# AnnaUshnova/tinyrenderder

Hardware: AMD Instinct MI355X
Metric: triangles/sec (+ Mpixels/sec) at 4096x4096; achieved HBM GB/s vs peak (higher is better)
Workload: dtype f64

## Files before the change

tinyrenderder_amd/csrc/kernels_bin.hip:

```cpp
#include <hip/hip_runtime.h>
#include "trgl_device.h"
#include "launch.h"

namespace {

__device__ __forceinline__ double dmin3(double a, double b, double c) { double m = a; if (b < m) m = b; if (c < m) m = c; return m; }
__device__ __forceinline__ double dmax3(double a, double b, double c) { double m = a; if (m < b) m = b; if (m < c) m = c; return m; }
__device__ __forceinline__ double dot4(const double* m, const double* v) {
    double sum = 0;
    sum += m[0] * v[0]; sum += m[1] * v[1]; sum += m[2] * v[2]; sum += m[3] * v[3];
    return sum;
}

__device__ __forceinline__ int wave_min_i(int v) {
    for (int o = 32; o; o >>= 1) { int t = __shfl_xor(v, o); v = t < v ? t : v; }
    return v;
}
__device__ __forceinline__ int wave_max_i(int v) {
    for (int o = 32; o; o >>= 1) { int t = __shfl_xor(v, o); v = t > v ? t : v; }
    return v;
}

constexpr int SCAN_THREADS = 256;

// ... 35 lines not shown
            if (++tx > tx1) { tx = tx0; ++row; ty = fp.il_tiles ? (uint32_t)il_nth_owned_from(fp, (int)ty0, (int)row) : ty0 + row; }
        }
    }
    unsigned long long big = __ballot(c > SMALL);
    const int lane = threadIdx.x & 63;
    while (big) {
        int src = __ffsll((long long)big) - 1;
        big &= big - 1;
        uint32_t cc = __shfl(c, src), oo = __shfl(o, src), ii = __shfl(i, src);
        uint32_t bx = __shfl(tb.x, src), by = __shfl(tb.y, src);
        const uint32_t qx0 = bx & 0x1fff, qy0 = (bx >> 16) & 0x1fff, qx1 = by & 0x1fff, qy1 = (by >> 16) & 0x1fff;
        ii |= (((bx >> 13) & 7u) | (((by >> 13) & 7u) << 3) | ((by >> 29) << 6)) << 25;
        uint32_t tx0 = qx0 >> 2, ty0 = qy0 >> 2, tx1 = qx1 >> 2;
        uint32_t wdt = tx1 - tx0 + 1;
        for (uint32_t k = lane; k < cc; k += 64) {
            uint32_t ty = fp.il_tiles ? (uint32_t)il_nth_owned_from(fp, (int)ty0, (int)(k / wdt)) : ty0 + k / wdt, tx = tx0 + k % wdt;
            put(oo + k, ty * tiles_x + tx, ii, tile_block_mask(tx, ty, qx0, qy0, qx1, qy1));
        }
    }
}

constexpr uint32_t SEG_MAX = 4096, SEG_MAX_GROUP = 16;

constexpr int SETUP_THREADS = 256;

__global__ __launch_bounds__(SETUP_THREADS) void k_setup(FrameParams fp, DrawDesc d, DrawDesc* __restrict__ draws_out, int draw_idx,
                                                         TriRec* __restrict__ recs, TriW* __restrict__ recs_w, uint32_t* __restrict__ cnt,
                                                         uint2* __restrict__ tilebox, DevStats* __restrict__ stats,
                                                         uint32_t* __restrict__ blk_sums, uint32_t blk_base,
                                                         uint32_t* __restrict__ seg_k, uint32_t* __restrict__ seg_v, uint32_t seg_S) {
    __shared__ __attribute__((aligned(16))) double s_buf[SETUP_THREADS * 16];
    if (blockIdx.x == 0 && threadIdx.x == 0) draws_out[draw_idx] = d;
    const uint32_t b0 = blockIdx.x * SETUP_THREADS;
    const uint32_t nb = min((uint32_t)SETUP_THREADS, d.n - b0);
    const uint32_t tid = threadIdx.x;
    const uint32_t i = b0 + tid;
    const bool in_range = tid < nb;

    const double* src = d.clip + (size_t)b0 * 12;
    if ((reinterpret_cast<uintptr_t>(src) & 15) == 0) {
        const double2* s2 = reinterpret_cast<const double2*>(src);
        double2* l2 = reinterpret_cast<double2*>(s_buf);
        typedef double f64x2 __attribute__((ext_vector_type(2)));
        for (uint32_t k = tid; k < nb * 6; k += SETUP_THREADS)
            *reinterpret_cast<f64x2*>(&l2[k]) = __builtin_nontemporal_load(reinterpret_cast<const f64x2*>(&s2[k]));
    } else {
        for (uint32_t k = tid; k < nb * 12; k += SETUP_THREADS) s_buf[k] = src[k];
    }
    __syncthreads();
    double v[12];
#pragma unroll
    for (int k = 0; k < 12; ++k) v[k] = in_range ? s_buf[tid * 12 + k] : 0.0;
    __syncthreads();

    int bx0 = INT_MAX, by0 = INT_MAX, bx1 = INT_MIN, by1 = INT_MIN;
    uint32_t ntiles = 0;
    bool large = false;
    uint2 tb = make_uint2(0, 0);
    TriRec r;
    {
        uint4* z4 = reinterpret_cast<uint4*>(&r);
#pragma unroll
        for (int k = 0; k < 8; ++k) z4[k] = make_uint4(0, 0, 0, 0);
    }
    if (in_range) {
        bool ok = !(v[3] <= 1e-12 || v[7] <= 1e-12 || v[11] <= 1e-12);
        double ndc[12];
#pragma unroll
        for (int q = 0; q < 3; ++q) {
#pragma unroll
            for (int k = 0; k < 3; ++k) ndc[4 * q + k] = v[4 * q + k] / v[4 * q + 3];
            ndc[4 * q + 3] = __builtin_isfinite(v[4 * q + 3]) ? 1.0 : __builtin_nan("");
        }
        bool zo0 = (ndc[2] < -1.0 || ndc[2] > 1.0), zo1 = (ndc[6] < -1.0 || ndc[6] > 1.0),
             zo2 = (ndc[10] < -1.0 || ndc[10] > 1.0);
        ok = ok && !(zo0 && zo1 && zo2);
#pragma unroll
        for (int k = 0; k < 12; ++k) ok = ok && __builtin_isfinite(ndc[k]);
        double sx[3], sy[3];
#pragma unroll
        for (int q = 0; q < 3; ++q) { sx[q] = dot4(fp.vp, ndc + 4 * q); sy[q] = dot4(fp.vp + 4, ndc + 4 * q); }
        double e1x = sx[1] - sx[0], e1y = sy[1] - sy[0], e2x = sx[2] - sx[0], e2y = sy[2] - sy[0];
// ... 8 lines not shown
            bx0 = min_x_px; by0 = min_y_px; bx1 = max_x_px; by1 = max_y_px;
            r.ax = sx[0]; r.ay = sy[0];
            r.s0x = sx[2] - sx[0]; r.s0y = sx[1] - sx[0];
            r.s1x = sy[2] - sy[0]; r.s1y = sy[1] - sy[0];
            r.uz = r.s0x * r.s1y - r.s0y * r.s1x;
            {
                const double BIG = 0x1p200, SMALL = 0x1p-250;
                bool ws = r.uz < 0.0 && !(fabs(r.uz) < 1e-12);
#pragma unroll
                for (int q = 0; q < 3; ++q) ws = ws && fabs(sx[q]) < BIG && fabs(sy[q]) < BIG;
                const double dl[4] = { r.s0x, r.s0y, r.s1x, r.s1y };
#pragma unroll
                for (int q = 0; q < 4; ++q) ws = ws && (dl[q] == 0.0 || fabs(dl[q]) >= SMALL);
                {
                    const double S = (fabs(r.s0x) + fabs(r.s0y)) + (fabs(r.s1x) + fabs(r.s1y));
                    const double rx = fmax(fabs(r.ax - ((double)bx0 + 0.5)), fabs(r.ax - ((double)bx1 + 0.5)));
                    const double ry = fmax(fabs(r.ay - ((double)by0 + 0.5)), fabs(r.ay - ((double)by1 + 0.5)));
                    ws = ws && 0x1p-40 * (S * S) * (rx + ry + 17.0 + S) < fabs(r.uz);
                }
                r.ruz = ws ? 1.0 / r.uz : 0.0;
            }
            r.z0 = ndc[2]; r.z1 = ndc[6]; r.z2 = ndc[10];
            r.bx0 = (uint16_t)bx0; r.by0 = (uint16_t)by0; r.bx1 = (uint16_t)bx1; r.by1 = (uint16_t)by1;
            r.color = d.colors ? d.colors[i] : 0xffffffffu;
            r.dl = ((uint32_t)draw_idx << 24) | i | (r.ruz == 0.0 ? TRGL_DL_LITERAL : 0u);
            r.c0 = -__builtin_inf(); r.g1 = 0.0; r.g2 = 0.0;
            if (r.ruz != 0.0) {
                const double zabs = dmax3(fabs(r.z0), fabs(r.z1), fabs(r.z2));
                const double dz1 = r.z1 - r.z0, dz2 = r.z2 - r.z0;
                const double h1 = (r.s1x * dz1 - r.s1y * dz2) * r.ruz, h2 = (r.s0y * dz2 - r.s0x * dz1) * r.ruz;
                const double rx = fmax(fabs(r.ax - ((double)bx0 + 0.5)), fabs(r.ax - ((double)bx1 + 0.5)));
                const double ry = fmax(fabs(r.ay - ((double)by0 + 0.5)), fabs(r.ay - ((double)by1 + 0.5)));
                const double Ssum = (fabs(r.s0x) + fabs(r.s0y)) + (fabs(r.s1x) + fabs(r.s1y));
                const double R = rx + ry + 1.0 + Ssum;
                const double mz = zabs * 0x1p-39 * (R * Ssum * fabs(r.ruz) + 1.0) + 0x1p-600;
                const bool okp = zabs < 0x1p1000 && R * fabs(h1) < 0x1p900 && R * fabs(h2) < 0x1p900 && mz < 0x1p1000;
                if (okp) { r.c0 = r.z0 - mz; r.g1 = h1; r.g2 = h2; }
            }
            if (d.kind != TRGL_SHADER_FLAT) {
                TriW w;
                w.iw0 = (fabs(v[3]) > 1e-12) ? (1.0 / v[3]) : 0.0;
                w.iw1 = (fabs(v[7]) > 1e-12) ? (1.0 / v[7]) : 0.0;
                w.iw2 = (fabs(v[11]) > 1e-12) ? (1.0 / v[11]) : 0.0;
                w.pad = 0.0;
                recs_w[d.first + i] = w;
            }
            int y_lo = max(by0, fp.strip_y0), y_hi = min(by1, fp.strip_y1 - 1);
            if (!(fabs(r.uz) < 1e-12) && y_lo <= y_hi) {
                uint32_t tx0 = bx0 >> TRGL_TILE_LOG2, tx1 = bx1 >> TRGL_TILE_LOG2;
                uint32_t ty0 = y_lo >> TRGL_TILE_LOG2, ty1 = y_hi >> TRGL_TILE_LOG2;
                const uint32_t rows = fp.il_tiles ? (uint32_t)(il_owned_below(fp, (int)ty1 + 1) - il_owned_below(fp, (int)ty0)) : ty1 - ty0 + 1;
                ntiles = (tx1 - tx0 + 1) * rows;
                tb = make_uint2(((uint32_t)bx0 >> TRGL_BLOCK_LOG2) | (((uint32_t)y_lo >> TRGL_BLOCK_LOG2) << 16),
                                ((uint32_t)bx1 >> TRGL_BLOCK_LOG2) | (((uint32_t)y_hi >> TRGL_BLOCK_LOG2) << 16));
                uint32_t zq = 0;
                if (r.c0 > -__builtin_inf()) {
                    const double zv = dmin3(r.c0, __builtin_fma(-r.s0y, r.g1, __builtin_fma(-r.s1y, r.g2, r.c0)),
                                            __builtin_fma(-r.s0x, r.g1, __builtin_fma(-r.s1x, r.g2, r.c0)));
                    const double t = (zv + 1.0) * 64.0 - 0x1p-20;
                    if (t >= 1.0) zq = t >= 127.0 ? 127u : (uint32_t)x86_cvttsd2si(floor(t));
                }
                tb.x |= (zq & 7u) << 13; tb.y |= ((zq >> 3) & 7u) << 13; tb.y |= (zq >> 6) << 29;
                large = ntiles != 0 && (bx1 - bx0 >= 64 || y_hi - y_lo >= 64);
            }
        }
        cnt[d.first + i] = ntiles;
        tilebox[d.first + i] = tb;
    }
    const uint32_t lane = tid & 63, wbase = tid & ~63u;
    {
        uint4* l4 = reinterpret_cast<uint4*>(s_buf);
        const uint4* r4 = reinterpret_cast<const uint4*>(&r);
#pragma unroll
        for (int c = 0; c < 8; ++c) l4[tid * 8 + (c ^ (tid & 7))] = r4[c];
        const unsigned long long keep = __ballot(ntiles != 0);
        __builtin_amdgcn_wave_barrier();
        uint4* dst = reinterpret_cast<uint4*>(recs + d.first + b0 + wbase);
#pragma unroll
        for (int it = 0; it < 8; ++it) {
            const uint32_t k = lane + 64u * it, t = k >> 3, c = k & 7;
            if ((keep >> t) & 1ull) {
                typedef uint32_t u32x4 __attribute__((ext_vector_type(4)));
                __builtin_nontemporal_store(*reinterpret_cast<const u32x4*>(&l4[(wbase + t) * 8 + (c ^ (t & 7))]), reinterpret_cast<u32x4*>(&dst[k]));
            }
        }
    }
    {
        const unsigned long long lit = __ballot(ntiles != 0 && r.ruz == 0.0);
        if (lit && lane == 0) atomicAdd(&stats->literal_tris, (unsigned long long)__popcll(lit));
        const unsigned long long lrg = __ballot(large);
        if (lrg && lane == 0) atomicAdd(&stats->large_tris, (unsigned long long)__popcll(lrg));
// ... 1 lines not shown
    int wx0 = wave_min_i(bx0), wy0 = wave_min_i(by0), wx1 = wave_max_i(bx1), wy1 = wave_max_i(by1);
    if ((threadIdx.x & 63) == 0 && wx0 != INT_MAX) {
        if (wx0 < __builtin_nontemporal_load(&stats->min_x)) atomicMin(&stats->min_x, wx0);
        if (wy0 < __builtin_nontemporal_load(&stats->min_y)) atomicMin(&stats->min_y, wy0);
        if (wx1 > __builtin_nontemporal_load(&stats->max_x)) atomicMax(&stats->max_x, wx1);
        if (wy1 > __builtin_nontemporal_load(&stats->max_y)) atomicMax(&stats->max_y, wy1);
    }
    uint32_t tot;
    const uint32_t off = block_excl_scan(ntiles, reinterpret_cast<uint32_t*>(s_buf), &tot);
    if (tid == 0) blk_sums[blk_base + blockIdx.x] = tot;
    if (seg_S && tot && tot <= seg_S) {
        __syncthreads();
        uint32_t* const s_k = reinterpret_cast<uint32_t*>(s_buf);
        uint32_t* const s_v = s_k + SEG_MAX;
        block_pairs(fp, fp.tiles_x, d.first + i, ntiles, tb, off, [&](uint32_t j, uint32_t key, uint32_t iz, uint32_t m) { s_k[j] = key | (m << 16); s_v[j] = iz; });
        __syncthreads();
        uint4* const kq = reinterpret_cast<uint4*>(seg_k + (size_t)(blk_base + blockIdx.x) * seg_S);
        uint4* const vq = reinterpret_cast<uint4*>(seg_v + (size_t)(blk_base + blockIdx.x) * seg_S);
        for (uint32_t q = tid; 4 * q < tot; q += SETUP_THREADS) {
            kq[q] = *reinterpret_cast<const uint4*>(s_k + 4 * q);
            vq[q] = *reinterpret_cast<const uint4*>(s_v + 4 * q);
        }
    }
}

constexpr int EXPAND_CHUNK = 16;

constexpr int SPINE_THREADS = 1024;
__global__ __launch_bounds__(SPINE_THREADS) void k_chunk_spine(const uint32_t* __restrict__ blk_sums, uint32_t nblk,
                                                               uint32_t* __restrict__ chunk_off,
                                                               unsigned long long* __restrict__ total64, unsigned long long* __restrict__ host_copy,
                                                               uint4* __restrict__ bounds16, uint32_t n_half16,
                                                               uint32_t seg_S, uint32_t seg_G, uint32_t seg_chunk,
                                                               uint32_t* __restrict__ seg_flag, uint32_t* __restrict__ seg_flag_host) {
    __shared__ unsigned long long s_wave[SPINE_THREADS / 64];
    int seg_bad = seg_S == 0;
    if (seg_S && seg_G != EXPAND_CHUNK) {
        for (uint32_t g = threadIdx.x; (uint64_t)g * seg_G < nblk; g += SPINE_THREADS) {
            uint32_t t[EXPAND_CHUNK];
#pragma unroll
            for (uint32_t k = 0; k < EXPAND_CHUNK; ++k) { const uint32_t q = g * seg_G + k; t[k] = (k < seg_G && q < nblk) ? blk_sums[q] : 0u; }
            unsigned long long sum = 0;
#pragma unroll
            for (uint32_t k = 0; k < EXPAND_CHUNK; ++k) sum += t[k];
            seg_bad |= sum > seg_chunk;
        }
// ... 82 lines not shown
        const uint32_t end = sh + tot;
        for (uint32_t q = threadIdx.x; 4 * q < end; q += 256) {
            const uint32_t j0 = 4 * q;
            if (j0 >= sh && j0 + 4 <= end) {
                *reinterpret_cast<uint4*>(kq + j0) = *reinterpret_cast<const uint4*>(s_k + j0);
                *reinterpret_cast<uint4*>(vq + j0) = *reinterpret_cast<const uint4*>(s_v + j0);
                if (WIDE) *reinterpret_cast<uint2*>(mq + j0) = *reinterpret_cast<const uint2*>(s_m + j0);
            } else {
                for (uint32_t j = j0; j < j0 + 4; ++j)
                    if (j >= sh && j < end) { kq[j] = s_k[j]; vq[j] = s_v[j]; if (WIDE) mq[j] = s_m[j]; }
            }
        }
    }
}

constexpr int RADIX_ROUNDS = 16;
constexpr int RADIX_WAVE_CHUNK = RADIX_ROUNDS * 64;
constexpr uint32_t RADIX_BIG_CAP = 4u << 20;
constexpr int RADIX_MAX_BITS = 8;

__global__ __launch_bounds__(256) void k_radix_hist(const uint32_t* __restrict__ keys, const unsigned long long* __restrict__ pairs_total,
                                                    uint32_t cap, int shift, int bits, uint32_t chunk,
                                                    uint32_t nblocks, uint32_t* __restrict__ hist, const uint32_t* __restrict__ skip) {
    __shared__ uint32_t s_cnt[1 << RADIX_MAX_BITS];
    const unsigned long long P64 = *pairs_total;
    const uint32_t P = (P64 > cap || (skip && *skip)) ? 0u : (uint32_t)P64;
    const uint32_t nb = 1u << bits, mask = nb - 1;
    for (uint32_t b = threadIdx.x; b < nb; b += 256) s_cnt[b] = 0;
    __syncthreads();
    const uint64_t beg = (uint64_t)blockIdx.x * chunk;
    uint64_t end = beg + chunk; if (end > P) end = P;
    for (uint64_t p = beg + 4u * threadIdx.x; p < end; p += 1024) {
        const uint4 q = *reinterpret_cast<const uint4*>(keys + p);
        const uint32_t k[4] = { q.x, q.y, q.z, q.w };
#pragma unroll
        for (int j = 0; j < 4; ++j) if (p + j < end) atomicAdd(&s_cnt[(k[j] >> shift) & mask], 1u);
    }
    __syncthreads();
    for (uint32_t b = threadIdx.x; b < nb; b += 256) hist[(size_t)b * nblocks + blockIdx.x] = s_cnt[b];
}

struct SegIn { const uint32_t* blk_sums; const uint32_t* flag; uint32_t nsetup, S, G; };

__global__ __launch_bounds__(256) void k_radix_hist_seg(const uint32_t* __restrict__ seg_k, SegIn seg, const unsigned long long* __restrict__ pairs_total,
                                                        uint32_t cap, int shift, int bits, uint32_t nblocks, uint32_t* __restrict__ hist) {
    __shared__ uint32_t s_cnt[1 << RADIX_MAX_BITS];
    const bool live = *seg.flag == 0 && *pairs_total <= cap;
    const uint32_t nb = 1u << bits, mask = nb - 1;
    for (uint32_t b = threadIdx.x; b < nb; b += 256) s_cnt[b] = 0;
    __syncthreads();
    const uint32_t w = threadIdx.x >> 6, lane = threadIdx.x & 63;
    if (live) {
        static_assert(SEG_MAX_GROUP == 16, "four waves of four segments");
        auto count4 = [&](const uint4 q, uint32_t p, uint32_t n) {
            const uint32_t k[4] = { q.x, q.y, q.z, q.w };
#pragma unroll
            for (int j = 0; j < 4; ++j) if (p + j < n) atomicAdd(&s_cnt[(k[j] >> shift) & mask], 1u);
        };
        uint32_t n[4]; const uint32_t* keys[4]; uint4 q[4][2];
#pragma unroll
        for (int j = 0; j < 4; ++j) {
            const uint32_t sg = w + 4 * j, b = blockIdx.x * seg.G + sg;
            const bool has = sg < seg.G && b < seg.nsetup;
            n[j] = has ? min(seg.blk_sums[b], seg.S) : 0u;
            keys[j] = seg_k + (size_t)(has ? b : 0u) * seg.S;
        }
#pragma unroll
        for (int j = 0; j < 4; ++j)
#pragma unroll
            for (int it = 0; it < 2; ++it) {
                const uint32_t p = 4 * lane + 256 * it;
                q[j][it] = p < n[j] ? *reinterpret_cast<const uint4*>(keys[j] + p) : make_uint4(0, 0, 0, 0);
            }
#pragma unroll
        for (int j = 0; j < 4; ++j) {
#pragma unroll
            for (int it = 0; it < 2; ++it) count4(q[j][it], 4 * lane + 256 * it, n[j]);
            for (uint32_t p = 512 + 4 * lane; p < n[j]; p += 256) count4(*reinterpret_cast<const uint4*>(keys[j] + p), p, n[j]);
        }
    }
    __syncthreads();
    for (uint32_t b = threadIdx.x; b < nb; b += 256) hist[(size_t)b * nblocks + blockIdx.x] = s_cnt[b];
}

constexpr int ROWSCAN_THREADS = 1024, ROWSCAN_PER = 8;
__global__ __launch_bounds__(ROWSCAN_THREADS) void k_radix_scan_rows(uint32_t* __restrict__ hist, uint32_t nblocks, uint32_t* __restrict__ totals) {
    __shared__ uint32_t s_wave[ROWSCAN_THREADS / 64];
    uint32_t* row = hist + (size_t)blockIdx.x * nblocks;
    const int lane = threadIdx.x & 63, w = threadIdx.x >> 6;
    uint32_t running = 0;
    for (uint32_t start = 0; start < nblocks; start += ROWSCAN_THREADS * ROWSCAN_PER) {
        const uint32_t base = start + threadIdx.x * ROWSCAN_PER;
        uint32_t v[ROWSCAN_PER], sum = 0;
#pragma unroll
        for (int k = 0; k < ROWSCAN_PER; ++k) { v[k] = (base + k < nblocks) ? row[base + k] : 0; sum += v[k]; }
        uint32_t inc = sum;
        for (int o = 1; o < 64; o <<= 1) { const uint32_t t = __shfl_up(inc, o); if (lane >= o) inc += t; }
        if (lane == 63) s_wave[w] = inc;
        __syncthreads();
        uint32_t wbase = 0, tot = 0;
#pragma unroll
        for (int k = 0; k < ROWSCAN_THREADS / 64; ++k) { const uint32_t t = s_wave[k]; if (k < w) wbase += t; tot += t; }
        uint32_t run = running + wbase + inc - sum;
#pragma unroll
        for (int k = 0; k < ROWSCAN_PER; ++k) { if (base + k < nblocks) row[base + k] = run; run += v[k]; }
// ... 167 lines not shown
        } else {
            msk_out[dst] = WIDE ? s_msk[i] : (uint16_t)(word >> 16);
            const uint32_t key = word & KEY_MASK;
            if (i == 0 || (s_key[i - 1] & KEY_MASK) != key) atomicMin(&tile_start[key], dst);
            if (i + 1 == n_chunk || (s_key[i + 1] & KEY_MASK) != key) atomicMax(&tile_end[key], dst + 1);
        }
    }
}

}

namespace trgl {

uint32_t setup_num_blocks(uint32_t n) { return (n + SETUP_THREADS - 1) / SETUP_THREADS; }

void launch_setup(hipStream_t s, const FrameParams& fp, const DrawDesc& draw, DrawDesc* draws_dev, int draw_idx, uint32_t n,
                  TriRec* recs, TriW* recs_w, uint32_t* cnt, uint2* tilebox, DevStats* stats, uint32_t* blk_sums, uint32_t blk_base,
                  const SegLayout* seg) {
    if (!n) return;
    hipLaunchKernelGGL(k_setup, dim3(setup_num_blocks(n)), dim3(SETUP_THREADS), 0, s, fp, draw, draws_dev, draw_idx, recs, recs_w, cnt, tilebox,
                       stats, blk_sums, blk_base, seg ? seg->keys : nullptr, seg ? seg->vals : nullptr, seg ? seg->S : 0u);
}

void launch_chunk_spine(hipStream_t s, const uint32_t* blk_sums, uint32_t nblk, uint32_t* chunk_off, unsigned long long* total64, unsigned long long* host_copy,
                        uint32_t* tile_bounds, size_t half_words, uint32_t seg_S, uint32_t seg_G, uint32_t seg_chunk, uint32_t* seg_flag,
                        uint32_t* seg_flag_host) {
    hipLaunchKernelGGL(k_chunk_spine, dim3(1), dim3(SPINE_THREADS), 0, s, blk_sums, nblk, chunk_off, total64, host_copy, (uint4*)tile_bounds,
                       (uint32_t)(half_words / 4), seg_S, seg_G, seg_chunk, seg_flag, seg_flag_host);
}

void launch_expand(hipStream_t s, const FrameParams& fp, uint32_t first, uint32_t n, int tiles_x, const uint32_t* cnt, const uint32_t* blk_sums,
                   const uint32_t* chunk_off, uint32_t blk_base, const uint2* tilebox, uint32_t* keys, bool wide, uint32_t* vals, uint16_t* bmask,
                   const unsigned long long* pairs_total, uint32_t cap) {
    if (!n) return;
    if (wide)
        hipLaunchKernelGGL(k_expand<true>, dim3(setup_num_blocks(n)), dim3(SETUP_THREADS), 0, s, fp, first, n, tiles_x, cnt, blk_sums, chunk_off,
                           blk_base, tilebox, keys, vals, bmask, pairs_total, cap);
    else
        hipLaunchKernelGGL(k_expand<false>, dim3(setup_num_blocks(n)), dim3(SETUP_THREADS), 0, s, fp, first, n, tiles_x, cnt, blk_sums, chunk_off,
                           blk_base, tilebox, keys, vals, bmask, pairs_total, cap);
}

static uint32_t radix_waves(uint32_t cap) { return cap >= RADIX_BIG_CAP ? 8u : 4u; }
uint32_t radix_chunk(uint32_t cap) { return radix_waves(cap) * RADIX_WAVE_CHUNK; }
uint32_t radix_num_workers(uint32_t cap) { const uint64_t chunk = radix_chunk(cap); return (uint32_t)((cap + chunk - 1) / chunk); }
uint32_t seg_num_groups(const SegLayout& seg) { return (seg.nsetup + seg.G - 1) / seg.G; }
// ... 40 lines not shown
```

tinyrenderder_amd/csrc/launch.h:

```cpp
#pragma once
#include <hip/hip_runtime.h>
#include "trgl_device.h"
#include "clip_core.h"

namespace trgl {

struct SegLayout { uint32_t* keys; uint32_t* vals; const uint32_t* blk_sums; const uint32_t* flag; uint32_t nsetup, S, G; };
bool seg_layout_ok(const SegLayout& seg);
uint32_t seg_num_groups(const SegLayout& seg);

uint32_t setup_num_blocks(uint32_t n);
void launch_setup(hipStream_t s, const FrameParams& fp, const DrawDesc& draw, DrawDesc* draws_dev, int draw_idx, uint32_t n,
                  TriRec* recs, TriW* recs_w, uint32_t* cnt, uint2* tilebox, DevStats* stats, uint32_t* blk_sums, uint32_t blk_base,
                  const SegLayout* seg);
void launch_chunk_spine(hipStream_t s, const uint32_t* blk_sums, uint32_t nblk, uint32_t* chunk_off, unsigned long long* total64, unsigned long long* host_copy,
                        uint32_t* tile_bounds, size_t half_words, uint32_t seg_S, uint32_t seg_G, uint32_t seg_chunk, uint32_t* seg_flag,
                        uint32_t* seg_flag_host);


void launch_expand(hipStream_t s, const FrameParams& fp, uint32_t first, uint32_t n, int tiles_x, const uint32_t* cnt, const uint32_t* blk_sums,
                   const uint32_t* chunk_off, uint32_t blk_base, const uint2* tilebox, uint32_t* keys, bool wide, uint32_t* vals, uint16_t* bmask,
                   const unsigned long long* pairs_total, uint32_t cap);

uint32_t radix_num_workers(uint32_t cap);
uint32_t radix_chunk(uint32_t cap);
struct RadixPass {
    const uint32_t* keys_in; const uint32_t* vals_in; const uint16_t* msk_in;
    uint32_t* keys_out; uint32_t* vals_out; uint16_t* msk_out;
    uint32_t* tile_start; uint32_t* tile_end;
    int shift, bits;
};
void launch_radix_pass(hipStream_t s, const RadixPass& ps, bool wide, bool last, const unsigned long long* pairs_total, uint32_t cap,
                       uint32_t* hist, uint32_t* scan_tmp, const SegLayout* seg = nullptr, const uint32_t* skip = nullptr);

uint32_t owned_tiles(const FrameParams& fp);
uint32_t raster_max_items(const FrameParams& fp);
struct UserShade { hipFunction_t fn; int kind; };
// ... 58 lines not shown
```

tinyrenderder_amd/csrc/trgl_api.cpp:

```cpp
#include <algorithm>
#include <cstring>

#include "trgl_ctx.h"
#include "user_shaders.h"

static size_t pair_capacity(size_t need) {
    const size_t ncap = (headroom(need) + 3) & ~size_t(3);
    return ncap > 0xffffe000ull ? 0xffffe000ull : ncap;
}

int trgl::fail(trgl_ctx* c, int code, const std::string& msg) { if (c) c->err = msg; else set_global_error(msg); return code; }

static int reset_dev_stats(trgl_ctx* c) {
    DevStats s;
    s.fragments = 0;
    s.zmin_key = zkey(std::numeric_limits<double>::infinity());
    s.zmax_key = zkey(-std::numeric_limits<double>::infinity());
    s.min_x = INT32_MAX; s.min_y = INT32_MAX; s.max_x = INT32_MIN; s.max_y = INT32_MIN;
    s.pairs_total = 0; s.literal_tris = 0; s.large_tris = 0;
    s.zero_pos_key = s.zero_neg_key = TRGL_ZERO_KEY_EMPTY;
    s.zero_locked = 0; s.zero_sign = 0;
    for (int k = 0; k < 16; ++k) s.dbg[k] = 0;
    *c->stats_pinned = s;
    HIPCHK(c, hipMemcpyAsync(c->stats_dev.p, c->stats_pinned, sizeof(DevStats), hipMemcpyHostToDevice, c->stream));
// ... 225 lines not shown
    return TRGL_OK;
}

static int resolve_events(trgl_ctx* c) {
    if (!c->events_pending) return TRGL_OK;
    HIPCHK(c, hipEventSynchronize(c->ev[3]));
    float ms;
    HIPCHK(c, hipEventElapsedTime(&ms, c->ev[0], c->ev[1])); c->phase_ms[TRGL_PHASE_SETUP] += ms;
    HIPCHK(c, hipEventElapsedTime(&ms, c->ev[1], c->ev[2])); c->phase_ms[TRGL_PHASE_BIN] += ms;
    HIPCHK(c, hipEventElapsedTime(&ms, c->ev[2], c->ev[3])); c->phase_ms[TRGL_PHASE_RASTER] += ms;
    HIPCHK(c, hipEventElapsedTime(&ms, c->ev[0], c->ev[3])); c->phase_ms[TRGL_PHASE_TOTAL] += ms;
    HIPCHK(c, hipEventElapsedTime(&ms, c->ev[4], c->ev[5])); c->phase_ms[TRGL_PHASE_RASTER_KERNEL] += ms;
    c->flushes_timed++;
    c->events_pending = false;
    return TRGL_OK;
}

int trgl_flush(trgl_ctx* c) {
    CHKCTX(c);
    int r = trgl_flush_begin(c);
    return r ? r : trgl_flush_end(c);
}

static int queue_binning(trgl_ctx* c, const FrameParams& fp, uint32_t cap, int* cur_out, const SegLayout* seg) {
    hipStream_t s = c->stream;
    const size_t ntiles = (size_t)c->tiles_x * c->tiles_y;
    const unsigned long long* pairs_dev = &c->stats_dev.p->pairs_total;
    int r;
    uint32_t blk_base = 0;
    const bool wide = ntiles > 65536;
    for (auto& d : c->draws) {
        if (seg) break;
        launch_expand(s, fp, d.first, d.n, c->tiles_x, c->cnt.p, c->blk_sums.p, c->chunk_off.p, blk_base, c->tilebox.p, c->keys[0].p, wide, c->vals[0].p,
                      c->bmask[0].p, pairs_dev, cap);
        blk_base += setup_num_blocks(d.n);
    }
    int key_bits = 1; while ((size_t(1) << key_bits) < ntiles) ++key_bits;
    int passes = (key_bits + 7) / 8;
    int bits_per = (key_bits + passes - 1) / passes;
    size_t hist_need = ((size_t)std::max(radix_num_workers(cap), seg ? seg_num_groups(*seg) : 0u) << bits_per) + 16;
    if ((r = c->hist.grow(c, hist_need))) return r;
    if ((r = c->scan_tmp.grow(c, 256 + 16))) return r;
    int cur = 0;
    for (int ps = 0; ps < passes; ++ps) {
        const RadixPass rp{ c->keys[cur].p, c->vals[cur].p, c->bmask[cur].p, c->keys[cur ^ 1].p, c->vals[cur ^ 1].p, c->bmask[cur ^ 1].p,
                            c->tile_start.p, c->tile_end(), ps * bits_per, bits_per };
// ... 15 lines not shown

static bool seg_sizes(double avg, uint32_t chunk, uint32_t* S, uint32_t* G) {
    if (avg < 1.0) avg = 1.0;
    const uint64_t s = ((uint64_t)(avg * 1.5) + 128 + 63) & ~uint64_t(63);
    uint64_t g = (uint64_t)(0.9 * chunk / avg);
    if (g > 16) g = 16;
    if (s > 4096 || g < 2) return false;
    *S = (uint32_t)s; *G = (uint32_t)g;
    return true;
}
constexpr uint64_t SEG_MAX_BYTES = uint64_t(1) << 30;

static int settle_binning(trgl_ctx* c, bool may_grow) {
    PendingRaster& rp = c->rp;
    if (!rp.N || rp.settled) return TRGL_OK;
    HIPCHK(c, hipEventSynchronize(c->ev_pairs));
    const unsigned long long P64 = c->stats_pinned->pairs_total;
    if (P64 > 0xffffe000ull) return TRGL_OK;
    const bool bad = *c->seg_flag_pinned != 0, over = P64 > rp.cap, fell = rp.direct && bad;
    if (over && !may_grow) return TRGL_OK;
    int r;
    if (over || fell) {
        if (over && (r = grow_pairs(c, (size_t)P64))) return r;
        if ((r = queue_binning(c, rp.fp, (uint32_t)c->keys[0].cap, &rp.cur, fell ? nullptr : (rp.direct ? &rp.seg : nullptr)))) return r;
        rp.cap = (uint32_t)c->keys[0].cap;
        if (c->profiling) HIPCHK(c, hipEventRecord(c->ev[2], c->stream));
    }
    if (c->bin_mode == 0) { if (fell) c->seg_hold = true; else if (!rp.direct && !bad) c->seg_hold = false; }
    rp.fell_back = fell; rp.settled = true;
    return TRGL_OK;
}

static FrameParams frame_params(const trgl_ctx* c) {
    FrameParams fp; std::memset(&fp, 0, sizeof(fp));
    fp.fb = c->fb.p; fp.zb = c->zb.p; fp.W = c->W; fp.H = c->H; fp.bpp = c->bpp;
    fp.tiles_x = c->tiles_x; fp.tiles_y = c->tiles_y;
    fp.strip_y0 = c->strip_y0; fp.strip_y1 = c->strip_y1;
    fp.strip_ty0 = c->strip_y0 / TRGL_TILE;
    fp.strip_ty1 = (c->strip_y1 + TRGL_TILE - 1) / TRGL_TILE;
    if (c->strip_y1 <= c->strip_y0) fp.strip_ty1 = fp.strip_ty0;
    fp.il_tiles = c->il_tiles; fp.il_world = c->il_world; fp.il_rank = c->il_rank;
    fp.init_from_clear = c->clear_pending ? 1 : 0;
    fp.n_tris = (uint32_t)c->queued_tris;
    fp.clear_color = c->clear_color; fp.clear_z = c->clear_z;
    std::memcpy(fp.vp, c->vp, sizeof(fp.vp));
    return fp;
// ... 26 lines not shown

    if (c->profiling) HIPCHK(c, hipEventRecord(c->ev[0], s));
    uint32_t cap = 0;
    int cur = 0;
    if (N) {
        const size_t tcap = headroom(N);
        if ((r = c->recs.grow(c, N + 1, tcap)) || (r = c->recs_w.grow(c, N + 1, tcap)) || (r = c->cnt.grow(c, N + 1, tcap)) ||
            (r = c->tilebox.grow(c, N + 1, tcap))) return r;
        if (c->keys[0].cap == 0 && (r = grow_pairs(c, (size_t)2 * N + 4096))) return r;
        uint32_t nblk = 0;
        for (auto& d : c->draws) nblk += setup_num_blocks(d.n);
        if ((r = c->blk_sums.grow(c, (size_t)nblk + 16))) return r;
        if ((r = c->chunk_off.grow(c, (size_t)nblk / 16 + 16))) return r;
        cap = (uint32_t)c->keys[0].cap;
        uint32_t S = 0, G = 0;
        bool direct = false;
        if ((size_t)c->tiles_x * c->tiles_y <= 65536) {
            if (c->bin_mode == 2) { S = c->bin_S; G = c->bin_G; direct = true; }
            else if (c->bin_mode == 0 && seg_sizes(c->rule_nblk ? (double)c->rule_pairs / (double)c->rule_nblk : 512.0, radix_chunk(cap), &S, &G))
                direct = !c->seg_hold && (uint64_t)nblk * S * 8 <= SEG_MAX_BYTES;
        }
        if (direct && ((r = c->seg_keys.grow(c, (size_t)nblk * S + 4)) || (r = c->seg_vals.grow(c, (size_t)nblk * S + 4)))) return r;
        const SegLayout seg{ c->seg_keys.p, c->seg_vals.p, c->blk_sums.p, c->seg_flag.p, nblk, S, G };
        c->rp.direct = direct; c->rp.seg = seg; c->rp.nblk = nblk;
        {
            uint32_t blk_base = 0;
            for (size_t i = 0; i < c->draws.size(); ++i) {
                launch_setup(s, fp, c->draws[i], c->draws_dev.p, (int)i, c->draws[i].n, c->recs.p, c->recs_w.p, c->cnt.p, c->tilebox.p, c->stats_dev.p,
                             c->blk_sums.p, blk_base, direct ? &seg : nullptr);
                blk_base += setup_num_blocks(c->draws[i].n);
            }
        }
        if (c->profiling) HIPCHK(c, hipEventRecord(c->ev[1], s));
        launch_chunk_spine(s, c->blk_sums.p, nblk, c->chunk_off.p, &c->stats_dev.p->pairs_total, &c->stats_pinned->pairs_total,
                           c->tile_start.p, c->bounds_half(), S, G, radix_chunk(cap), c->seg_flag.p, c->seg_flag_pinned);
        HIPCHK(c, hipEventRecord(c->ev_pairs, s));
        if ((r = queue_binning(c, fp, cap, &cur, direct ? &seg : nullptr))) return r;
    } else {
        c->rp.direct = false; c->rp.nblk = 0; c->rp.seg = SegLayout{};
        if (c->profiling) HIPCHK(c, hipEventRecord(c->ev[1], s));
        HIPCHK(c, hipMemsetAsync(c->tile_start.p, 0, c->bounds_half() * 8, s));
    }
    if (c->profiling) HIPCHK(c, hipEventRecord(c->ev[2], s));
    c->rp.active = true; c->rp.fp = fp; c->rp.flush_kind = flush_kind; c->rp.cap = cap; c->rp.cur = cur; c->rp.N = N;
    c->rp.builtin_shade = builtin_shade; c->rp.user_kinds = user_kinds;
    c->rp.settled = false; c->rp.fell_back = false;
    return TRGL_OK;
}

int trgl_flush_end(trgl_ctx* c) {
    CHKCTX(c);
    if (!c->rp.active) return TRGL_OK;
    c->rp.active = false;
    int r;
    hipStream_t s = c->stream;
    FrameParams fp = c->rp.fp;
    const int flush_kind = c->rp.flush_kind;
    int cur = c->rp.cur;
    const uint64_t N = c->rp.N;
    uint32_t P = 0;
    if (N) {
        HIPCHK(c, hipEventSynchronize(c->ev_pairs));
// ... 12 lines not shown
    const uint32_t max_items = raster_max_items(fp);
    if ((r = c->items.grow(c, (size_t)max_items + 64))) return r;
    if ((r = c->item_stats.grow(c, ((size_t)max_items + 64) * 4))) return r;
    const bool all_well_scaled = N == 0 || c->stats_pinned->literal_tris == 0;
    fp.zq_cull = (N != 0 && c->stats_pinned->large_tris != 0) ? 1 : 0;
    UserShade user[TRGL_MAX_USER_SHADERS];
    int n_user = 0;
    for (int i = 0; i < (int)c->user.size(); ++i)
        if (c->rp.user_kinds >> i & 1u) user[n_user++] = UserShade{ c->user[i].fn, TRGL_SHADER_USER_FIRST + i };
    const hipFunction_t user_raster = discarding_kind(c, flush_kind) ? user_kind(c, flush_kind)->fn : nullptr;
    launch_raster(s, fp, flush_kind, all_well_scaled, recs_arg, c->recs_w.p, vals_arg, bmask_arg, c->tile_start.p, c->tile_end(), c->draws_dev.p, c->tex_dev.p,
                  c->stats_dev.p, max_items, c->items.p, c->n_items.p, c->item_stats.p, c->rp.builtin_shade, user, n_user, user_raster,
                  c->profiling ? c->ev[4] : nullptr, c->profiling ? c->ev[5] : nullptr);
    if (c->profiling) { HIPCHK(c, hipEventRecord(c->ev[3], s)); c->events_pending = true; }
    HIPCHK(c, hipGetLastError());

    c->triangles_total += N;
    if (N) { c->rule_pairs = P; c->rule_nblk = c->rp.nblk; }
    c->snap = Snapshot{ true, c->rp, P, N ? c->stats_pinned->literal_tris : 0, N ? c->stats_pinned->large_tris : 0 };
    c->snap.rp.fp = fp; c->snap.rp.cap = (uint32_t)c->keys[0].cap;
    c->clear_pending = false;
    bool had_stage = false;
    for (auto& ch : c->stage) if (ch.used) had_stage = true;
    c->draws.clear();
    c->queued_tris = 0;
    if (had_stage) {
        HIPCHK(c, hipStreamSynchronize(s));
        if (!c->stage_hold)
            for (auto& ch : c->stage) ch.used = 0;
    }
    return TRGL_OK;
}

int trgl_sync(trgl_ctx* c) {
    CHKCTX(c);
    int r = end_pending_raster(c); if (r) return r;
    HIPCHK(c, hipStreamSynchronize(c->stream));
    return TRGL_OK;
}

int trgl_read_framebuffer(trgl_ctx* c, uint8_t* dst) {
    CHKCTX(c);
    if (!dst) return fail(c, TRGL_E_INVALID, "null destination");
    int r = flush_sync(c); if (r) return r;
    HIPCHK(c, hipMemcpy(dst, c->fb.p, (size_t)c->W * c->H * c->bpp, hipMemcpyDeviceToHost));
    return TRGL_OK;
// ... 100 lines not shown
        }
        f.rp.fp.zq_cull = f.large_tris != 0 ? 1 : 0;
    }
    const FrameParams& fp = f.rp.fp; const uint64_t N = f.rp.N, P = f.P, cap = f.rp.cap; const int cur = f.rp.cur;
    const size_t ntiles = (size_t)c->tiles_x * c->tiles_y;
    if (what >= 3 && what <= 6 && P > cap) return fail(c, TRGL_E_STATE, "trgl_debug_read: the pending flush has more pairs than the pair buffers hold; its lists exist after trgl_flush_end");
    int64_t info[24] = { (int64_t)N, (int64_t)P, (int64_t)cap, ntiles > 65536 ? 1 : 0, (int64_t)f.literal_tris, (int64_t)f.large_tris, fp.zq_cull, pending ? 1 : 0,
                         fp.W, fp.H, fp.tiles_x, fp.tiles_y, fp.strip_y0, fp.strip_y1, fp.strip_ty0, fp.strip_ty1, fp.il_tiles, fp.il_world, fp.il_rank, cur, f.rp.direct, f.rp.fell_back, f.rp.seg.S, f.rp.seg.G };
    const void* src = nullptr; size_t need = 0;
    switch (what) {
    case 0: src = c->recs.p; need = N ? (size_t)(N + 1) * sizeof(TriRec) : 0; break;
    case 1: src = c->cnt.p; need = (size_t)N * sizeof(uint32_t); break;
    case 2: src = c->tilebox.p; need = (size_t)N * sizeof(uint2); break;
    case 3: src = c->vals[cur].p; need = (size_t)P * sizeof(uint32_t); break;
    case 4: src = c->bmask[cur].p; need = (size_t)P * sizeof(uint16_t); break;
    case 5: src = c->tile_start.p; need = ntiles * sizeof(uint32_t); break;
    case 6: src = c->tile_end(); need = ntiles * sizeof(uint32_t); break;
    default: need = sizeof(info); break;
    }
    if (needed) *needed = need;
    if (!dst) return TRGL_OK;
    if (bytes < need) return fail(c, TRGL_E_INVALID, "trgl_debug_read: destination too small");
    if (what == 7) { std::memcpy(dst, info, sizeof(info)); return TRGL_OK; }
    HIPCHK(c, hipStreamSynchronize(c->stream));
    if (need) HIPCHK(c, hipMemcpy(dst, src, need, hipMemcpyDeviceToHost));
    return TRGL_OK;
}

extern "C" int trgl_debug_binning(trgl_ctx* c, int mode, uint32_t S, uint32_t G, int* last_direct, int* last_fell_back) {
    CHKCTX(c);
    if (mode < -1 || mode > 2) return fail(c, TRGL_E_INVALID, "trgl_debug_binning: mode is -1 (report only), 0 (automatic), 1 (k_expand) or 2 (direct)");
    if (mode == 2 && !seg_layout_ok(SegLayout{ nullptr, nullptr, nullptr, nullptr, 0, S, G }))
        return fail(c, TRGL_E_INVALID, "trgl_debug_binning: S is a multiple of 4 in 4..4096, G in 1..16");
    if (mode >= 0) { c->bin_mode = mode; c->bin_S = mode == 2 ? S : 0; c->bin_G = mode == 2 ? G : 0; c->seg_hold = false; }
    if (last_direct) *last_direct = c->snap.rp.direct;
    if (last_fell_back) *last_fell_back = c->snap.rp.fell_back;
    return TRGL_OK;
}

int trgl_get_last_flush_info(trgl_ctx* c, uint64_t* triangles, uint64_t* pairs, uint64_t* tiles) {
    if (!c) return TRGL_E_INVALID;
    if (triangles) *triangles = c->snap.rp.N;
    if (pairs) *pairs = c->snap.P;
    if (tiles) *tiles = (uint64_t)c->tiles_x * c->tiles_y;
    return TRGL_OK;
}
// ... 3 lines not shown
```

tinyrenderder_amd/csrc/trgl_ctx.h:

```cpp
#pragma once
#include <hip/hip_runtime.h>

#include <limits>
#include <string>
#include <vector>

#include "../../include/trgl.h"
#include "launch.h"
#include "trgl_device.h"

namespace trgl {
struct StageChunk { char* base; size_t cap, used; };

inline size_t headroom(size_t need) { return need + need / 4 + 1024; }
template <class T> struct DevBuf {
    T* p = nullptr;
    size_t cap = 0;
    DevBuf() = default;
    DevBuf(const DevBuf&) = delete;
    ~DevBuf() { if (p) (void)hipFree(p); }
    int alloc(trgl_ctx* c, size_t n);
    int grow(trgl_ctx* c, size_t need, size_t ncap) { return need <= cap ? TRGL_OK : alloc(c, ncap); }
    int grow(trgl_ctx* c, size_t need) { return grow(c, need, headroom(need)); }
    int release(trgl_ctx* c);
};

struct PendingRaster { bool active = false; FrameParams fp; int flush_kind = 0; uint32_t cap = 0; int cur = 0; uint64_t N = 0;
                       bool builtin_shade = false; uint32_t user_kinds = 0;
                       bool direct = false, settled = false, fell_back = false; SegLayout seg{}; uint32_t nblk = 0; };
struct Snapshot { bool valid = false; PendingRaster rp; uint64_t P = 0, literal_tris = 0, large_tris = 0; };
struct UserKind { hipModule_t mod; hipFunction_t fn; int K; bool may_discard; };
struct UserVertex { hipModule_t mod; hipFunction_t fn; int K; };
}
using namespace trgl;

struct trgl_ctx {
    int device = 0;
    int W = 0, H = 0, bpp = 0, tiles_x = 0, tiles_y = 0;
    hipStream_t stream = nullptr;
    hipStream_t own_stream = nullptr;
    DevBuf<uint8_t> fb;
    DevBuf<double> zb;
    double vp[16];
    bool clear_pending = true;
    uint32_t clear_color = 0xff000000u;
    double clear_z = std::numeric_limits<double>::infinity();
    int strip_y0 = 0, strip_y1 = 0;
    int il_tiles = 0, il_world = 1, il_rank = 0;

    DevTexture tex_host[TRGL_MAX_TEXTURES];
    DevBuf<DevTexture> tex_dev;

// ... 12 lines not shown
    DevBuf<float> blur_weights; DevBuf<uint8_t> blur_tmp; int blur_radius = 0;
    float* blur_w_pinned = nullptr; size_t blur_w_pinned_cap = 0; hipEvent_t ev_blur_w = nullptr;
    DevBuf<uint32_t> clip_scratch;
    DevBuf<uint8_t> shadow_tmp;
    DevBuf<uint8_t> pp_out;
    DevBuf<uint32_t> blk_sums;
    DevBuf<uint32_t> chunk_off;
    DevBuf<uint32_t> keys[2], vals[2]; DevBuf<uint16_t> bmask[2];
    DevBuf<uint32_t> hist, scan_tmp;
    DevBuf<uint32_t> seg_keys, seg_vals, seg_flag;
    uint32_t* seg_flag_pinned = nullptr;
    int bin_mode = 0; uint32_t bin_S = 0, bin_G = 0;
    bool seg_hold = false;
    uint64_t rule_pairs = 0, rule_nblk = 0;
    DevBuf<uint32_t> tile_start;
    DevBuf<uint4> items; DevBuf<uint32_t> n_items;
    DevBuf<unsigned long long> item_stats;
    DevBuf<DrawDesc> draws_dev;
    DevBuf<DevStats> stats_dev;
    DevStats* stats_pinned = nullptr;

    uint64_t triangles_total = 0;
    Snapshot snap;

    bool profiling = false, events_pending = false;
    hipEvent_t ev[6] = { nullptr, nullptr, nullptr, nullptr, nullptr, nullptr };
    double phase_ms[TRGL_NUM_PHASES] = { 0, 0, 0, 0, 0 };
    uint64_t flushes_timed = 0;

    std::vector<UserKind> user;
    std::vector<UserVertex> vertex;

    std::string err;

    size_t bounds_half() const { return ((size_t)tiles_x * tiles_y + 3) & ~size_t(3); }
    uint32_t* tile_end() const { return tile_start.p + bounds_half(); }
};

#define HIPCHK(ctx, expr)                                                                      \
    do {                                                                                       \
        hipError_t e_ = (expr);                                                                \
        if (e_ != hipSuccess) {                                                                \
            (ctx)->err = std::string(#expr) + ": " + hipGetErrorString(e_);                    \
            return TRGL_E_HIP;                                                                 \
        }                                                                                      \
    } while (0)
// ... 38 lines not shown
```

Before: 4.222 billion.

## Skip per-triangle count/tilebox stores in direct segmented binning; recompute lazily

In the direct segmented binning path, the setup kernel no longer writes the per-triangle tile counts and tile boxes. A new k_tile_counts kernel recomputes them on demand, either when binning falls back or when debug reads request them, and the previous frame's draws are kept so they can be regenerated. The setup math is factored into a templated device function to support this. The radix histogram kernels also get per-wave privatized shared-memory counters and batched key loads to cut atomic contention. This trades HBM store traffic in the common case for extra recompute on the fallback and debug paths.

```diff
diff --git a/tinyrenderder_amd/csrc/kernels_bin.hip b/tinyrenderder_amd/csrc/kernels_bin.hip
--- a/tinyrenderder_amd/csrc/kernels_bin.hip
+++ b/tinyrenderder_amd/csrc/kernels_bin.hip
@@ -81,42 +81,16 @@
 
 constexpr uint32_t SEG_MAX = 4096, SEG_MAX_GROUP = 16;
 
-constexpr int SETUP_THREADS = 256;
-
-__global__ __launch_bounds__(SETUP_THREADS) void k_setup(FrameParams fp, DrawDesc d, DrawDesc* __restrict__ draws_out, int draw_idx,
-                                                         TriRec* __restrict__ recs, TriW* __restrict__ recs_w, uint32_t* __restrict__ cnt,
-                                                         uint2* __restrict__ tilebox, DevStats* __restrict__ stats,
-                                                         uint32_t* __restrict__ blk_sums, uint32_t blk_base,
-                                                         uint32_t* __restrict__ seg_k, uint32_t* __restrict__ seg_v, uint32_t seg_S) {
-    __shared__ __attribute__((aligned(16))) double s_buf[SETUP_THREADS * 16];
-    if (blockIdx.x == 0 && threadIdx.x == 0) draws_out[draw_idx] = d;
-    const uint32_t b0 = blockIdx.x * SETUP_THREADS;
-    const uint32_t nb = min((uint32_t)SETUP_THREADS, d.n - b0);
-    const uint32_t tid = threadIdx.x;
-    const uint32_t i = b0 + tid;
-    const bool in_range = tid < nb;
-
-    const double* src = d.clip + (size_t)b0 * 12;
-    if ((reinterpret_cast<uintptr_t>(src) & 15) == 0) {
-        const double2* s2 = reinterpret_cast<const double2*>(src);
-        double2* l2 = reinterpret_cast<double2*>(s_buf);
-        typedef double f64x2 __attribute__((ext_vector_type(2)));
-        for (uint32_t k = tid; k < nb * 6; k += SETUP_THREADS)
-            *reinterpret_cast<f64x2*>(&l2[k]) = __builtin_nontemporal_load(reinterpret_cast<const f64x2*>(&s2[k]));
-    } else {
-        for (uint32_t k = tid; k < nb * 12; k += SETUP_THREADS) s_buf[k] = src[k];
-    }
-    __syncthreads();
-    double v[12];
-#pragma unroll
-    for (int k = 0; k < 12; ++k) v[k] = in_range ? s_buf[tid * 12 + k] : 0.0;
-    __syncthreads();
-
+struct SetupTri { TriRec r; uint32_t ntiles; uint2 tb; bool large; int bx0, by0, bx1, by1; };
+
+template <bool RECORD>
+__device__ __forceinline__ void setup_triangle(const FrameParams& fp, const DrawDesc& d, int draw_idx, uint32_t i, bool in_range,
+                                               const double (&v)[12], TriW* __restrict__ recs_w, SetupTri& t) {
     int bx0 = INT_MAX, by0 = INT_MAX, bx1 = INT_MIN, by1 = INT_MIN;
     uint32_t ntiles = 0;
     bool large = false;
     uint2 tb = make_uint2(0, 0);
-    TriRec r;
+    TriRec& r = t.r;
     {
         uint4* z4 = reinterpret_cast<uint4*>(&r);
 #pragma unroll
@@ -171,7 +145,7 @@
             }
             r.z0 = ndc[2]; r.z1 = ndc[6]; r.z2 = ndc[10];
             r.bx0 = (uint16_t)bx0; r.by0 = (uint16_t)by0; r.bx1 = (uint16_t)bx1; r.by1 = (uint16_t)by1;
-            r.color = d.colors ? d.colors[i] : 0xffffffffu;
+            r.color = (RECORD && d.colors) ? d.colors[i] : 0xffffffffu;
             r.dl = ((uint32_t)draw_idx << 24) | i | (r.ruz == 0.0 ? TRGL_DL_LITERAL : 0u);
             r.c0 = -__builtin_inf(); r.g1 = 0.0; r.g2 = 0.0;
             if (r.ruz != 0.0) {
@@ -186,7 +160,7 @@
                 const bool okp = zabs < 0x1p1000 && R * fabs(h1) < 0x1p900 && R * fabs(h2) < 0x1p900 && mz < 0x1p1000;
                 if (okp) { r.c0 = r.z0 - mz; r.g1 = h1; r.g2 = h2; }
             }
-            if (d.kind != TRGL_SHADER_FLAT) {
+            if (RECORD && d.kind != TRGL_SHADER_FLAT) {
                 TriW w;
                 w.iw0 = (fabs(v[3]) > 1e-12) ? (1.0 / v[3]) : 0.0;
                 w.iw1 = (fabs(v[7]) > 1e-12) ? (1.0 / v[7]) : 0.0;
@@ -213,9 +187,49 @@
                 large = ntiles != 0 && (bx1 - bx0 >= 64 || y_hi - y_lo >= 64);
             }
         }
-        cnt[d.first + i] = ntiles;
-        tilebox[d.first + i] = tb;
-    }
+    }
+    t.ntiles = ntiles; t.tb = tb; t.large = large; t.bx0 = bx0; t.by0 = by0; t.bx1 = bx1; t.by1 = by1;
+}
+
+constexpr int SETUP_THREADS = 256;
+
+__global__ __launch_bounds__(SETUP_THREADS) void k_setup(FrameParams fp, DrawDesc d, DrawDesc* __restrict__ draws_out, int draw_idx,
+                                                         TriRec* __restrict__ recs, TriW* __restrict__ recs_w, uint32_t* __restrict__ cnt,
+                                                         uint2* __restrict__ tilebox, DevStats* __restrict__ stats,
+                                                         uint32_t* __restrict__ blk_sums, uint32_t blk_base,
+                                                         uint32_t* __restrict__ seg_k, uint32_t* __restrict__ seg_v, uint32_t seg_S) {
+    __shared__ __attribute__((aligned(16))) double s_buf[SETUP_THREADS * 16];
+    if (blockIdx.x == 0 && threadIdx.x == 0) draws_out[draw_idx] = d;
+    const uint32_t b0 = blockIdx.x * SETUP_THREADS;
+    const uint32_t nb = min((uint32_t)SETUP_THREADS, d.n - b0);
+    const uint32_t tid = threadIdx.x;
+    const uint32_t i = b0 + tid;
+    const bool in_range = tid < nb;
+
+    const double* src = d.clip + (size_t)b0 * 12;
+    if ((reinterpret_cast<uintptr_t>(src) & 15) == 0) {
+        const double2* s2 = reinterpret_cast<const double2*>(src);
+        double2* l2 = reinterpret_cast<double2*>(s_buf);
+        typedef double f64x2 __attribute__((ext_vector_type(2)));
+        for (uint32_t k = tid; k < nb * 6; k += SETUP_THREADS)
+            *reinterpret_cast<f64x2*>(&l2[k]) = __builtin_nontemporal_load(reinterpret_cast<const f64x2*>(&s2[k]));
+    } else {
+        for (uint32_t k = tid; k < nb * 12; k += SETUP_THREADS) s_buf[k] = src[k];
+    }
+    __syncthreads();
+    double v[12];
+#pragma unroll
+    for (int k = 0; k < 12; ++k) v[k] = in_range ? s_buf[tid * 12 + k] : 0.0;
+    __syncthreads();
+
+    SetupTri t;
+    setup_triangle<true>(fp, d, draw_idx, i, in_range, v, recs_w, t);
+    const TriRec& r = t.r;
+    const uint32_t ntiles = t.ntiles;
+    const uint2 tb = t.tb;
+    const bool large = t.large;
+    const int bx0 = t.bx0, by0 = t.by0, bx1 = t.bx1, by1 = t.by1;
+    if (in_range && !seg_S) { cnt[d.first + i] = ntiles; tilebox[d.first + i] = tb; }
     const uint32_t lane = tid & 63, wbase = tid & ~63u;
     {
         uint4* l4 = reinterpret_cast<uint4*>(s_buf);
@@ -263,6 +277,18 @@
             vq[q] = *reinterpret_cast<const uint4*>(s_v + 4 * q);
         }
     }
+}
+
+__global__ __launch_bounds__(SETUP_THREADS) void k_tile_counts(FrameParams fp, DrawDesc d, int draw_idx, uint32_t* __restrict__ cnt,
+                                                               uint2* __restrict__ tilebox) {
+    const uint32_t i = blockIdx.x * SETUP_THREADS + threadIdx.x;
+    const bool in_range = i < d.n;
+    double v[12];
+#pragma unroll
+    for (int k = 0; k < 12; ++k) v[k] = in_range ? d.clip[(size_t)i * 12 + k] : 0.0;
+    SetupTri t;
+    setup_triangle<false>(fp, d, draw_idx, i, in_range, v, nullptr, t);
+    if (in_range) { cnt[d.first + i] = t.ntiles; tilebox[d.first + i] = t.tb; }
 }
 
 constexpr int EXPAND_CHUNK = 16;
@@ -391,32 +417,41 @@
 __global__ __launch_bounds__(256) void k_radix_hist(const uint32_t* __restrict__ keys, const unsigned long long* __restrict__ pairs_total,
                                                     uint32_t cap, int shift, int bits, uint32_t chunk,
                                                     uint32_t nblocks, uint32_t* __restrict__ hist, const uint32_t* __restrict__ skip) {
-    __shared__ uint32_t s_cnt[1 << RADIX_MAX_BITS];
+    constexpr int HIST_LOADS = 8;
+    static_assert(HIST_LOADS * 256 * 4 >= 8 * RADIX_WAVE_CHUNK, "a chunk of the largest radix block in one round of loads");
+    __shared__ uint32_t s_cnt[4][1 << RADIX_MAX_BITS];
     const unsigned long long P64 = *pairs_total;
     const uint32_t P = (P64 > cap || (skip && *skip)) ? 0u : (uint32_t)P64;
-    const uint32_t nb = 1u << bits, mask = nb - 1;
-    for (uint32_t b = threadIdx.x; b < nb; b += 256) s_cnt[b] = 0;
+    const uint32_t nb = 1u << bits, mask = nb - 1, w = threadIdx.x >> 6;
+    for (uint32_t b = threadIdx.x; b < nb; b += 256) { s_cnt[0][b] = 0; s_cnt[1][b] = 0; s_cnt[2][b] = 0; s_cnt[3][b] = 0; }
     __syncthreads();
     const uint64_t beg = (uint64_t)blockIdx.x * chunk;
     uint64_t end = beg + chunk; if (end > P) end = P;
-    for (uint64_t p = beg + 4u * threadIdx.x; p < end; p += 1024) {
-        const uint4 q = *reinterpret_cast<const uint4*>(keys + p);
-        const uint32_t k[4] = { q.x, q.y, q.z, q.w };
-#pragma unroll
-        for (int j = 0; j < 4; ++j) if (p + j < end) atomicAdd(&s_cnt[(k[j] >> shift) & mask], 1u);
-    }
-    __syncthreads();
-    for (uint32_t b = threadIdx.x; b < nb; b += 256) hist[(size_t)b * nblocks + blockIdx.x] = s_cnt[b];
+    uint4 q[HIST_LOADS];
+#pragma unroll
+    for (int it = 0; it < HIST_LOADS; ++it) {
+        const uint64_t p = beg + 4u * threadIdx.x + 1024u * it;
+        q[it] = p < end ? *reinterpret_cast<const uint4*>(keys + p) : make_uint4(0, 0, 0, 0);
+    }
+#pragma unroll
+    for (int it = 0; it < HIST_LOADS; ++it) {
+        const uint64_t p = beg + 4u * threadIdx.x + 1024u * it;
+        const uint32_t k[4] = { q[it].x, q[it].y, q[it].z, q[it].w };
+#pragma unroll
+        for (int j = 0; j < 4; ++j) if (p + j < end) atomicAdd(&s_cnt[w][(k[j] >> shift) & mask], 1u);
+    }
+    __syncthreads();
+    for (uint32_t b = threadIdx.x; b < nb; b += 256) hist[(size_t)b * nblocks + blockIdx.x] = (s_cnt[0][b] + s_cnt[1][b]) + (s_cnt[2][b] + s_cnt[3][b]);
 }
 
 struct SegIn { const uint32_t* blk_sums; const uint32_t* flag; uint32_t nsetup, S, G; };
 
 __global__ __launch_bounds__(256) void k_radix_hist_seg(const uint32_t* __restrict__ seg_k, SegIn seg, const unsigned long long* __restrict__ pairs_total,
                                                         uint32_t cap, int shift, int bits, uint32_t nblocks, uint32_t* __restrict__ hist) {
-    __shared__ uint32_t s_cnt[1 << RADIX_MAX_BITS];
+    __shared__ uint32_t s_cnt[4][1 << RADIX_MAX_BITS];
     const bool live = *seg.flag == 0 && *pairs_total <= cap;
     const uint32_t nb = 1u << bits, mask = nb - 1;
-    for (uint32_t b = threadIdx.x; b < nb; b += 256) s_cnt[b] = 0;
+    for (uint32_t b = threadIdx.x; b < nb; b += 256) { s_cnt[0][b] = 0; s_cnt[1][b] = 0; s_cnt[2][b] = 0; s_cnt[3][b] = 0; }
     __syncthreads();
     const uint32_t w = threadIdx.x >> 6, lane = threadIdx.x & 63;
     if (live) {
@@ -424,7 +459,7 @@
         auto count4 = [&](const uint4 q, uint32_t p, uint32_t n) {
             const uint32_t k[4] = { q.x, q.y, q.z, q.w };
 #pragma unroll
-            for (int j = 0; j < 4; ++j) if (p + j < n) atomicAdd(&s_cnt[(k[j] >> shift) & mask], 1u);
+            for (int j = 0; j < 4; ++j) if (p + j < n) atomicAdd(&s_cnt[w][(k[j] >> shift) & mask], 1u);
         };
         uint32_t n[4]; const uint32_t* keys[4]; uint4 q[4][2];
 #pragma unroll
@@ -449,7 +484,7 @@
         }
     }
     __syncthreads();
-    for (uint32_t b = threadIdx.x; b < nb; b += 256) hist[(size_t)b * nblocks + blockIdx.x] = s_cnt[b];
+    for (uint32_t b = threadIdx.x; b < nb; b += 256) hist[(size_t)b * nblocks + blockIdx.x] = (s_cnt[0][b] + s_cnt[1][b]) + (s_cnt[2][b] + s_cnt[3][b]);
 }
 
 constexpr int ROWSCAN_THREADS = 1024, ROWSCAN_PER = 8;
@@ -663,6 +698,11 @@
                        stats, blk_sums, blk_base, seg ? seg->keys : nullptr, seg ? seg->vals : nullptr, seg ? seg->S : 0u);
 }
 
+void launch_tile_counts(hipStream_t s, const FrameParams& fp, const DrawDesc& draw, int draw_idx, uint32_t* cnt, uint2* tilebox) {
+    if (!draw.n) return;
+    hipLaunchKernelGGL(k_tile_counts, dim3(setup_num_blocks(draw.n)), dim3(SETUP_THREADS), 0, s, fp, draw, draw_idx, cnt, tilebox);
+}
+
 void launch_chunk_spine(hipStream_t s, const uint32_t* blk_sums, uint32_t nblk, uint32_t* chunk_off, unsigned long long* total64, unsigned long long* host_copy,
                         uint32_t* tile_bounds, size_t half_words, uint32_t seg_S, uint32_t seg_G, uint32_t seg_chunk, uint32_t* seg_flag,
                         uint32_t* seg_flag_host) {
diff --git a/tinyrenderder_amd/csrc/launch.h b/tinyrenderder_amd/csrc/launch.h
--- a/tinyrenderder_amd/csrc/launch.h
+++ b/tinyrenderder_amd/csrc/launch.h
@@ -13,6 +13,7 @@
 void launch_setup(hipStream_t s, const FrameParams& fp, const DrawDesc& draw, DrawDesc* draws_dev, int draw_idx, uint32_t n,
                   TriRec* recs, TriW* recs_w, uint32_t* cnt, uint2* tilebox, DevStats* stats, uint32_t* blk_sums, uint32_t blk_base,
                   const SegLayout* seg);
+void launch_tile_counts(hipStream_t s, const FrameParams& fp, const DrawDesc& draw, int draw_idx, uint32_t* cnt, uint2* tilebox);
 void launch_chunk_spine(hipStream_t s, const uint32_t* blk_sums, uint32_t nblk, uint32_t* chunk_off, unsigned long long* total64, unsigned long long* host_copy,
                         uint32_t* tile_bounds, size_t half_words, uint32_t seg_S, uint32_t seg_G, uint32_t seg_chunk, uint32_t* seg_flag,
                         uint32_t* seg_flag_host);
diff --git a/tinyrenderder_amd/csrc/trgl_api.cpp b/tinyrenderder_amd/csrc/trgl_api.cpp
--- a/tinyrenderder_amd/csrc/trgl_api.cpp
+++ b/tinyrenderder_amd/csrc/trgl_api.cpp
@@ -271,6 +271,12 @@
     return r ? r : trgl_flush_end(c);
 }
 
+static void queue_tile_counts(trgl_ctx* c, PendingRaster& rp, const std::vector<DrawDesc>& draws) {
+    if (!rp.N || rp.counts_stored) return;
+    for (size_t i = 0; i < draws.size(); ++i) launch_tile_counts(c->stream, rp.fp, draws[i], (int)i, c->cnt.p, c->tilebox.p);
+    rp.counts_stored = true;
+}
+
 static int queue_binning(trgl_ctx* c, const FrameParams& fp, uint32_t cap, int* cur_out, const SegLayout* seg) {
     hipStream_t s = c->stream;
     const size_t ntiles = (size_t)c->tiles_x * c->tiles_y;
@@ -332,6 +338,7 @@
     int r;
     if (over || fell) {
         if (over && (r = grow_pairs(c, (size_t)P64))) return r;
+        if (fell) queue_tile_counts(c, rp, c->draws);
         if ((r = queue_binning(c, rp.fp, (uint32_t)c->keys[0].cap, &rp.cur, fell ? nullptr : (rp.direct ? &rp.seg : nullptr)))) return r;
         rp.cap = (uint32_t)c->keys[0].cap;
         if (c->profiling) HIPCHK(c, hipEventRecord(c->ev[2], c->stream));
@@ -404,7 +411,7 @@
         }
         if (direct && ((r = c->seg_keys.grow(c, (size_t)nblk * S + 4)) || (r = c->seg_vals.grow(c, (size_t)nblk * S + 4)))) return r;
         const SegLayout seg{ c->seg_keys.p, c->seg_vals.p, c->blk_sums.p, c->seg_flag.p, nblk, S, G };
-        c->rp.direct = direct; c->rp.seg = seg; c->rp.nblk = nblk;
+        c->rp.direct = direct; c->rp.counts_stored = !direct; c->rp.seg = seg; c->rp.nblk = nblk;
         {
             uint32_t blk_base = 0;
             for (size_t i = 0; i < c->draws.size(); ++i) {
@@ -419,7 +426,7 @@
         HIPCHK(c, hipEventRecord(c->ev_pairs, s));
         if ((r = queue_binning(c, fp, cap, &cur, direct ? &seg : nullptr))) return r;
     } else {
-        c->rp.direct = false; c->rp.nblk = 0; c->rp.seg = SegLayout{};
+        c->rp.direct = false; c->rp.counts_stored = true; c->rp.nblk = 0; c->rp.seg = SegLayout{};
         if (c->profiling) HIPCHK(c, hipEventRecord(c->ev[1], s));
         HIPCHK(c, hipMemsetAsync(c->tile_start.p, 0, c->bounds_half() * 8, s));
     }
@@ -478,6 +485,7 @@
     c->clear_pending = false;
     bool had_stage = false;
     for (auto& ch : c->stage) if (ch.used) had_stage = true;
+    c->snap_draws.swap(c->draws);
     c->draws.clear();
     c->queued_tris = 0;
     if (had_stage) {
@@ -624,6 +632,7 @@
     if (!dst) return TRGL_OK;
     if (bytes < need) return fail(c, TRGL_E_INVALID, "trgl_debug_read: destination too small");
     if (what == 7) { std::memcpy(dst, info, sizeof(info)); return TRGL_OK; }
+    if ((what == 1 || what == 2) && need) queue_tile_counts(c, pending ? c->rp : c->snap.rp, pending ? c->draws : c->snap_draws);
     HIPCHK(c, hipStreamSynchronize(c->stream));
     if (need) HIPCHK(c, hipMemcpy(dst, src, need, hipMemcpyDeviceToHost));
     return TRGL_OK;
diff --git a/tinyrenderder_amd/csrc/trgl_ctx.h b/tinyrenderder_amd/csrc/trgl_ctx.h
--- a/tinyrenderder_amd/csrc/trgl_ctx.h
+++ b/tinyrenderder_amd/csrc/trgl_ctx.h
@@ -27,7 +27,7 @@
 
 struct PendingRaster { bool active = false; FrameParams fp; int flush_kind = 0; uint32_t cap = 0; int cur = 0; uint64_t N = 0;
                        bool builtin_shade = false; uint32_t user_kinds = 0;
-                       bool direct = false, settled = false, fell_back = false; SegLayout seg{}; uint32_t nblk = 0; };
+                       bool direct = false, settled = false, fell_back = false, counts_stored = false; SegLayout seg{}; uint32_t nblk = 0; };
 struct Snapshot { bool valid = false; PendingRaster rp; uint64_t P = 0, literal_tris = 0, large_tris = 0; };
 struct UserKind { hipModule_t mod; hipFunction_t fn; int K; bool may_discard; };
 struct UserVertex { hipModule_t mod; hipFunction_t fn; int K; };
@@ -86,6 +86,7 @@
 
     uint64_t triangles_total = 0;
     Snapshot snap;
+    std::vector<DrawDesc> snap_draws;
 
     bool profiling = false, events_pending = false;
     hipEvent_t ev[6] = { nullptr, nullptr, nullptr, nullptr, nullptr, nullptr };
```

Measured after the change: 4.249 billion, median of 6. No clear change (+0.6%).
